# skyhehe123/SA-SSD

Measured on AMD Instinct MI355X. Metric: KITTI-Car inference frames/sec (whole job), higher is better.
Workload: dtype f32; 1 GPU; configs/car_cfg.py inference, fp32, synthetic lidar64 K21 frames (21500 pts -> ~16k voxels), batch=1, random-init SA-SSD weights, points resident in HBM; frames_in_flight=3, spconv_cfg=0, rulebook_pyramid=levels, launch=one hipGraph replay per frame, parallelism=frame-sharded x1, no collective

## Files before the change

### include/sassd.h

```cpp
#ifndef SASSD_H
#define SASSD_H

#include <stddef.h>
#include <stdint.h>

#ifdef __cplusplus
extern "C" {
#endif

#define SASSD_OK       0
#define SASSD_EINVAL  -1
#define SASSD_ENOSPC  -2
#define SASSD_EHIP    -3

#define SASSD_ST_VOXEL_OVERFLOW   1
#define SASSD_ST_HASH_FULL        2
#define SASSD_ST_BOX_OVERFLOW     4
#define SASSD_ST_GRID_SYNC        8

#define SASSD_MAX_POINTS_PER_VOXEL 64

const char *sassd_version(void);
int sassd_last_hip_error(void);
const char *sassd_last_hip_error_string(void);
// ... 88 lines not shown
int sassd_conv2d_wino_supported(int Cin, int Cout, int H, int W);
size_t sassd_conv2d_wino_packed_floats(int Cin, int Cout);
int sassd_conv2d_wino_pack_weight(const float *w, int Cout, int Cin, float *packed, void *stream);
int sassd_conv2d_wino_fwd(const float *x, const float *w_packed, const float *scale, const float *shift, int relu,
                          float *y, int batch, int Cin, int Cout, int H, int W, void *stream);

int sassd_conv2d_wino4_supported(int Cin, int Cout, int H, int W);
size_t sassd_conv2d_wino4_packed_floats(int Cin, int Cout);
int sassd_conv2d_wino4_pack_weight(const float *w , int Cout, int Cin, float *packed, void *stream);
size_t sassd_conv2d_wino4_workspace_bytes(int batch, int Cin, int Cout, int H, int W);
int sassd_conv2d_wino4_fwd(const float *x, const float *w_packed, const float *scale, const float *shift, int relu,
                           float *y, int batch, int Cin, int Cout, int H, int W, int cfg, void *workspace,
                           size_t workspace_bytes, void *stream);

int sassd_conv2d_wino4_chain_supported(int Cin, int Cout, int H, int W);
size_t sassd_conv2d_wino4_chain_workspace_bytes(int batch, int cmax, int H, int W);
int sassd_conv2d_wino4_chain(const float *x, int src_products, const float *prev_scale, const float *prev_shift,
                             int prev_relu, const float *w_packed, const float *scale, const float *shift, int relu,
                             float *y, int batch, int Cin, int Cout, int cmax, int H, int W, const int32_t *tile_map,
                             const int32_t *prev_tile_map, int cfg, void *workspace, size_t workspace_bytes,
                             void *stream);
size_t sassd_conv2d_wino4_narrow_packed_floats(int Cin);
int sassd_conv2d_wino4_pack_weight_narrow(const float *w , int Cout, int Cin, float *packed, void *stream);
int sassd_conv2d_wino4_chain_tail(const float *prev_scale, const float *prev_shift, int prev_relu, float *y_prev,
                                  const float *w_packed64, const float *scale, const float *shift, int relu, float *y,
                                  int batch, int Cin, int Cout, int cmax, int H, int W, const int32_t *prev_tile_map, int cfg,
                                  void *workspace, size_t workspace_bytes, void *stream);

size_t sassd_wino4_tile_map_ints(int batch, int H, int W);
int sassd_wino4_tile_map(const int32_t *indices, const int32_t *n_ptr, int cap, int batch, int H, int W,
                         int32_t *tile_map, void *stream);

int sassd_conv1x1_gemm_supported(int Cin, int Cout, int H, int W);
int sassd_conv1x1_gemm_pack_weight(const float *w , int Cout, int Cin, float *packed, void *stream);
int sassd_conv1x1_gemm_fwd(const float *x, const float *w_packed, const float *scale, const float *shift, int relu,
                           float *y, int batch, int Cin, int Cout, int H, int W, int cfg, void *stream);

int sassd_conv2d_bf16_supported(int Cin, int Cout, int H, int W);
size_t sassd_conv2d_bf16_packed_elems(int Cin, int Cout);
int sassd_conv2d_bf16_pack_weight(const float *w, int Cout, int Cin, void *packed, void *stream);
int sassd_conv2d_bf16_fwd(const float *x, const void *w_packed, const float *shift, float *y, int batch, int Cin,
                          int Cout, int H, int W, void *stream);
int sassd_conv2d_bf16_fwd_cfg(const float *x, const void *w_packed, const float *shift, float *y, int batch, int Cin,
                              int Cout, int H, int W, int cfg, void *stream);
int sassd_conv2d_bf16_bnrelu_fwd(const float *x, const float *in_affine, const void *w_packed, const float *shift, float *y,
                                 int batch, int Cin, int Cout, int H, int W, void *stream);

int sassd_conv1x1_bf16_supported(int Cin, int Cout, int HW);
size_t sassd_conv1x1_bf16_packed_elems(int Cin, int Cout);
int sassd_conv1x1_bf16_pack_weight(const float *w, int Cout, int Cin, int transposed, void *packed, void *stream);
int sassd_conv1x1_bf16_fwd(const float *x, const void *w_packed, const float *shift, float *y, int batch, int Cin, int Cout,
                           int HW, void *stream);

int sassd_conv2d_bf16_infer_supported(int Cin, int Cout, int H, int W);
size_t sassd_conv2d_bf16_infer_packed_elems(int Cin, int Cout);
int sassd_conv2d_bf16_infer_pack_weight(const float *w, int Cout, int Cin, void *packed, void *stream);
int sassd_conv2d_bf16_infer_fwd(const void *x, const void *w_packed, const float *scale, const float *shift, int relu, void *y,
                                int y_bf16, int batch, int Cin, int Cout, int H, int W, void *stream);
int sassd_conv1x1_bf16_infer_supported(int Cin, int Cout, int HW);
int sassd_conv1x1_bf16_infer_fwd(const void *x, const void *w_packed, const float *scale, const float *shift, int relu, void *y,
                                 int y_bf16, int batch, int Cin, int Cout, int HW, void *stream);

size_t sassd_conv2d_wgrad_workspace_bytes(int batch, int Cin, int Cout, int H, int W, int ksize);
int sassd_conv2d_bwd_weight(const float *x, const float *dy, float *dw, int batch, int Cin, int Cout, int H, int W,
                            int ksize, int accumulate, void *workspace, size_t workspace_bytes, void *stream);
int sassd_conv2d_bwd_weight_bf16(const float *x, const float *dy, float *dw, int batch, int Cin, int Cout, int H, int W,
// ... 179 lines not shown
```

### sa-ssd_amd/_C.py

```python
import ctypes as C
import os
import subprocess

_HERE = os.path.dirname(os.path.abspath(__file__))
LIB_PATH = os.path.join(_HERE, "lib", "libsassd.so")
_lib = None

OK, EINVAL, ENOSPC, EHIP = 0, -1, -2, -3
ST_VOXEL_OVERFLOW, ST_HASH_FULL, ST_BOX_OVERFLOW = 1, 2, 4


def build(force=False, verbose=False):
    cmd = ["make", "-C", os.path.join(_HERE, "csrc"), "-j8"]
    if force:
        subprocess.check_call(cmd + ["clean"], stdout=subprocess.DEVNULL)
    out = subprocess.run(cmd, stdout=subprocess.PIPE, stderr=subprocess.STDOUT, text=True)
    if verbose or out.returncode != 0:
        print(out.stdout)
    if out.returncode != 0:
        raise RuntimeError("building libsassd.so failed")
    return LIB_PATH


_SZ = C.c_size_t
# ... 41 lines not shown
    "sassd_conv2d_pack_weight": (_I, [_P, _I, _I, _I, _P, _P]),
    "sassd_conv2d_fwd": (_I, [_P, _P, _P, _P, _I, _P, _I, _I, _I, _I, _I, _I, _P]),
    "sassd_conv2d_fwd_cfg": (_I, [_P, _P, _P, _P, _I, _P, _I, _I, _I, _I, _I, _I, _I, _P]),
    "sassd_anchor_mask_workspace_bytes": (_SZ, [_I, _I]),
    "sassd_anchor_mask": (_I, [_P, _P, _P, _I, _I, _P, _I, _P, _P, _F, _P, _P, _SZ, _P]),
    "sassd_anchor_mask_batch": (_I, [_P, _P, _I, _I, _I, _P, _I, _P, _P, _F, _P, _P, _SZ, _P]),
    "sassd_decode_filter_workspace_bytes": (_SZ, [_I, _I]),
    "sassd_decode_filter": (_I, [_P, _P, _P, _SZ, _I, _I, _I, _I, _I, _P, _P, _F, _P, _P, _P, _P, _I, _P, _P, _SZ, _P]),
    "sassd_pswarp_sample": (_I, [_P, _I, _I, _I, _P, _P, _I, _F, _F, _F, _P, _P]),
    "sassd_pswarp_sample_bwd": (_I, [_P, _I, _I, _I, _P, _P, _I, _F, _F, _F, _P, _P, _P, _P]),
    "sassd_rescore_nms_workspace_bytes": (_SZ, [_I, _I]),
    "sassd_rescore_nms": (_I, [_P, _P, _P, _P, _I, _I, _F, _F, _P, _P, _P, _P, _I, _P, _P, _SZ, _P]),
    "sassd_boxes_overlap_bev": (_I, [_P, _I, _P, _I, _P, _P]),
    "sassd_boxes_iou_bev": (_I, [_P, _I, _P, _I, _P, _P]),
    "sassd_nms_workspace_bytes": (_SZ, [_I]),
    "sassd_nms_gpu": (_I, [_P, _I, _F, _P, _P, _P, _SZ, _P]),
    "sassd_nms_normal_gpu": (_I, [_P, _I, _F, _P, _P, _P, _SZ, _P]),
    "sassd_three_nn": (_I, [_I, _I, _P, _P, _P, _P, _P]),
    "sassd_three_interpolate": (_I, [_I, _I, _I, _P, _P, _P, _P, _P]),
    "sassd_three_interpolate_grad": (_I, [_I, _I, _I, _P, _P, _P, _P, _P]),
    "sassd_pts_in_boxes3d": (_I, [_P, _I, _P, _I, _P, _P, _P]),
    "sassd_three_nn_binned_workspace_bytes": (_SZ, [_I, _I, _I, _I]),
    "sassd_three_nn_binned": (_I, [_I, _I, _P, _P, _F, _F, _F, _I, _I, _I, _P, _P, _P, _SZ, _P]),
    "sassd_conv2d_wino_supported": (_I, [_I, _I, _I, _I]),
    "sassd_conv2d_wino_packed_floats": (_SZ, [_I, _I]),
    "sassd_conv2d_wino_pack_weight": (_I, [_P, _I, _I, _P, _P]),
    "sassd_conv2d_wino_fwd": (_I, [_P, _P, _P, _P, _I, _P, _I, _I, _I, _I, _I, _P]),
    "sassd_conv2d_wino4_supported": (_I, [_I, _I, _I, _I]),
    "sassd_conv2d_wino4_packed_floats": (_SZ, [_I, _I]),
    "sassd_conv2d_wino4_pack_weight": (_I, [_P, _I, _I, _P, _P]),
    "sassd_conv2d_wino4_workspace_bytes": (_SZ, [_I, _I, _I, _I, _I]),
    "sassd_conv2d_wino4_fwd": (_I, [_P, _P, _P, _P, _I, _P, _I, _I, _I, _I, _I, _I, _P, _SZ, _P]),
    "sassd_conv1x1_gemm_supported": (_I, [_I, _I, _I, _I]),
    "sassd_conv1x1_gemm_pack_weight": (_I, [_P, _I, _I, _P, _P]),
    "sassd_conv1x1_narrow_supported": (_I, [_I, _I]),
    "sassd_conv1x1_narrow_pad": (_I, [_I]),
    "sassd_conv1x1_narrow_fwd": (_I, [_P, _P, _P, _P, _I, _P, _I, _I, _I, _I, _I, _P]),
    "sassd_conv1x1_gemm_fwd": (_I, [_P, _P, _P, _P, _I, _P, _I, _I, _I, _I, _I, _I, _P]),
    "sassd_conv2d_bf16_supported": (_I, [_I, _I, _I, _I]),
    "sassd_conv2d_bf16_packed_elems": (_SZ, [_I, _I]),
    "sassd_conv2d_bf16_pack_weight": (_I, [_P, _I, _I, _P, _P]),
    "sassd_conv2d_bf16_fwd": (_I, [_P, _P, _P, _P, _I, _I, _I, _I, _I, _P]),
    "sassd_conv2d_bf16_fwd_cfg": (_I, [_P, _P, _P, _P, _I, _I, _I, _I, _I, _I, _P]),
    "sassd_conv2d_bf16_bnrelu_fwd": (_I, [_P, _P, _P, _P, _P, _I, _I, _I, _I, _I, _P]),
    "sassd_conv1x1_bf16_supported": (_I, [_I, _I, _I]),
    "sassd_conv1x1_bf16_packed_elems": (_SZ, [_I, _I]),
    "sassd_conv1x1_bf16_pack_weight": (_I, [_P, _I, _I, _I, _P, _P]),
    "sassd_conv1x1_bf16_fwd": (_I, [_P, _P, _P, _P, _I, _I, _I, _I, _P]),
    "sassd_conv2d_bf16_infer_supported": (_I, [_I, _I, _I, _I]),
    "sassd_conv2d_bf16_infer_packed_elems": (_SZ, [_I, _I]),
    "sassd_conv2d_bf16_infer_pack_weight": (_I, [_P, _I, _I, _P, _P]),
    "sassd_conv2d_bf16_infer_fwd": (_I, [_P, _P, _P, _P, _I, _P, _I, _I, _I, _I, _I, _I, _P]),
    "sassd_conv1x1_bf16_infer_supported": (_I, [_I, _I, _I]),
    "sassd_conv1x1_bf16_infer_fwd": (_I, [_P, _P, _P, _P, _I, _P, _I, _I, _I, _I, _I, _P]),
    "sassd_conv2d_wgrad_workspace_bytes": (_SZ, [_I, _I, _I, _I, _I, _I]),
    "sassd_conv2d_bwd_weight": (_I, [_P, _P, _P, _I, _I, _I, _I, _I, _I, _I, _P, _SZ, _P]),
    "sassd_assign_targets_workspace_bytes": (_SZ, [_I, _I, _I]),
    "sassd_assign_targets": (_I, [_P, _I, _P, _I, _I, _P, _P, _P, _P, _I, _P, _P, _F, _F, _P, _P, _P, _SZ, _P, _I, _P,
                                  _SZ, _P]),
    "sassd_guided_select_workspace_bytes": (_SZ, [_I, _I]),
    "sassd_guided_select": (_I, [_P, _P, _I, _I, _I, _F, _I, _P, _P, _P, _P, _SZ, _P]),
    "sassd_rpn_loss_workspace_bytes": (_SZ, [_I, _I]),
    "sassd_rpn_loss": (_I, [_P, _P, _P, _I, _P, _P, _P, _I, _P, _I, _I, _P, _P, _P, _P, _P, _SZ, _P]),
    "sassd_conv2d_bwd_weight_bf16": (_I, [_P, _P, _P, _I, _I, _I, _I, _I, _I, _I, _P, _SZ, _P]),
    "sassd_conv2d_bwd_weight_bf16_bnrelu": (_I, [_P, _P, _P, _P, _I, _I, _I, _I, _I, _I, _I, _P, _SZ, _P]),
    "sassd_rotate_iou_eval": (_I, [_P, _I, _P, _I, _I, _P, _P]),
# ... 92 lines not shown
```

### sa-ssd_amd/csrc/conv2d_wino4.hip

```cpp
#include "common.h"

namespace {
typedef float f32x16 __attribute__((ext_vector_type(16)));
typedef __bf16 bf16x8 __attribute__((ext_vector_type(8)));
typedef unsigned u32x4 __attribute__((ext_vector_type(4)));
typedef __attribute__((address_space(3))) void *lds_ptr_t;
typedef const __attribute__((address_space(1))) void *glb_ptr_t;

constexpr int kBM = 128, kKC = 32;

__device__ __forceinline__ void g_row(const float g0, const float g1, const float g2, float (&o)[6])
{
    o[0] = g0;
    const float e = g0 + 0.390625f * g2, f = 0.625f * g1;
    o[1] = e + f;
    o[2] = e - f;
    const float e2 = g0 + 2.25f * g2, f2 = 1.5f * g1;
    o[3] = e2 + f2;
    o[4] = e2 - f2;
    o[5] = g2;
}

__global__ void wino4_pack_kernel(const float *__restrict__ w, int Cout, int Cin, float *__restrict__ U, int ldu)
{
// ... 250 lines not shown
    }
}

static int launch_outin(int dbg, int Cin, int batch, size_t lds, hipStream_t stream, const float *M, W4Geom G,
                        const float *scale, const float *shift, int relu, int pitch, float *V, const int32_t *tmap,
                        float *y_prev)
{
    static std::atomic<unsigned long long> done512{0}, done256{0};
    if (dbg & 256) {
        int rc = sassd_dyn_lds((const void *)wino4_outin_kernel<256>, (size_t)160 * 1024, done256);
        if (rc) return rc;
        hipLaunchKernelGGL(wino4_outin_kernel<256>, dim3(Cin, batch), dim3(256), lds, stream, M, G, scale, shift, relu, pitch,
                           V, tmap, y_prev);
    } else {
        int rc = sassd_dyn_lds((const void *)wino4_outin_kernel<512>, (size_t)160 * 1024, done512);
        if (rc) return rc;
        hipLaunchKernelGGL(wino4_outin_kernel<512>, dim3(Cin, batch), dim3(512), lds, stream, M, G, scale, shift, relu, pitch,
                           V, tmap, y_prev);
    }
    return SASSD_OK;
}

struct W4Gemm {
    const float *U, *V;
    float *M;
    const float *scale, *shift;
    size_t su, sv, sm;
    int np, Cin, Cout, ldv, ldm, ncols, relu;
    int nmb, nnb;
    int nseg, seglen;
    int pairs_per_xcd;
    int dbg;
    const int32_t *ncols_dev;
};

__device__ __forceinline__ void split3(const float a, unsigned &u0, unsigned &u1, unsigned &u2)
{
    u0 = __float_as_uint(a);
    const float r1 = a - __uint_as_float(u0 & 0xffff0000u);
    u1 = __float_as_uint(r1);
    const float r2 = r1 - __uint_as_float(u1 & 0xffff0000u);
    u2 = __float_as_uint(r2);
}
__device__ __forceinline__ unsigned hi_pair(const unsigned lo, const unsigned hi)
{
    return __builtin_amdgcn_perm(hi, lo, 0x07060302u);
}
__device__ __forceinline__ bf16x8 split_a(const float a)
{
    unsigned u0, u1, u2;
    split3(a, u0, u1, u2);
    u32x4 d;
    d[0] = hi_pair(u0, u1); d[1] = hi_pair(u2, u0); d[2] = d[0]; d[3] = hi_pair(u1, u2);
    return __builtin_bit_cast(bf16x8, d);
}
__device__ __forceinline__ bf16x8 split_b(const float w)
{
    unsigned u0, u1, u2;
    split3(w, u0, u1, u2);
    u32x4 d;
    d[0] = hi_pair(u0, u0); d[1] = hi_pair(u0, u1); d[2] = hi_pair(u2, u1); d[3] = d[2];
    return __builtin_bit_cast(bf16x8, d);
}

template <int M, int NM, int NV>
__device__ __forceinline__ void split_sched()
// ... 137 lines not shown
                    for (int a = 0; a < MT; ++a) acc[a][b] = __builtin_amdgcn_mfma_f32_32x32x2f32(av[a], bv, acc[a][b], 0, 0, 0);
                }
            }
        }
        __syncthreads();
    }
    constexpr int WCOLS = 32 * NB;
    float *img = lds + wave * WROWS * WCOLS;
#pragma unroll
    for (int a = 0; a < MT; ++a)
#pragma unroll
        for (int b = 0; b < NB; ++b)
#pragma unroll
            for (int r = 0; r < 16; ++r)
                img[(a * 32 + (r & 3) + 8 * (r >> 2) + 4 * kh) * WCOLS + b * 32 + l31] = acc[a][b][r];
    asm volatile("s_waitcnt lgkmcnt(0)" ::: "memory");
    const int co0 = mb * BM + wm * WROWS;
    float *Mb = P.M + (size_t)p * P.sm + (size_t)co0 * P.ldm + nb * BN + wn * WCOLS;
    constexpr int C4 = WCOLS / 4, RPI = 64 / C4;
    const bool epi = P.scale || P.shift || P.relu;
#pragma unroll
    for (int i = 0; i < WROWS / RPI; ++i) {
        const int row = i * RPI + lane / C4, c4 = lane % C4;
        float4 v = *reinterpret_cast<const float4 *>(img + row * WCOLS + c4 * 4);
        if (epi) {
            const float sc = P.scale ? P.scale[co0 + row] : 1.f, sh = P.shift ? P.shift[co0 + row] : 0.f;
            v.x = v.x * sc + sh; v.y = v.y * sc + sh; v.z = v.z * sc + sh; v.w = v.w * sc + sh;
            if (P.relu) { v.x = fmaxf(v.x, 0.f); v.y = fmaxf(v.y, 0.f); v.z = fmaxf(v.z, 0.f); v.w = fmaxf(v.w, 0.f); }
        }
        *reinterpret_cast<float4 *>(Mb + (size_t)row * P.ldm + c4 * 4) = v;
    }
}

inline int w4_geo(int cfg) { return cfg & 0xff; }
inline int w4_dbg(int cfg) { return cfg >> 8; }

template <int WM, int WN, int NB, int KC, int SPLIT = 0>
int launch_w4_gemm(W4Gemm P, int dbg, hipStream_t stream)
{
    constexpr int BM = 64 * WM, BN = 32 * NB * WN;
    static_assert(BM == kBM || (WM == 1 && SPLIT != 0), "the channel block is fixed (w4_pick_wn and the supported() checks price "
                                                        "it); the one exception is the 64-channel block of a narrow tail layer");
    constexpr size_t stage_b = (size_t)2 * (BM + BN) * KC * 4, img_b = (size_t)WM * WN * 64 * 32 * NB * 4;
    constexpr size_t lds = stage_b > img_b ? stage_b : img_b;
    if constexpr (SPLIT == 1)
        if (dbg & 4) return launch_w4_gemm<WM, WN, NB, KC, 2>(P, dbg, stream);
    static std::atomic<unsigned long long> attr_done{0};
    const void *fn = (const void *)wino4_gemm_kernel<WM, WN, NB, KC, SPLIT>;
    int rc = sassd_dyn_lds(fn, lds, attr_done);
    if (rc) return rc;
    P.nmb = P.Cout / BM; P.nnb = P.ncols / BN;
    const int pairs = P.np * P.nmb;
    P.nseg = pairs >= 32 ? 1 : cdiv(32, pairs);
    if (P.nseg > P.nnb) P.nseg = P.nnb;
    P.seglen = cdiv(P.nnb, P.nseg);
    P.pairs_per_xcd = cdiv(pairs * P.nseg, 8);
    P.dbg = dbg;
    hipLaunchKernelGGL((wino4_gemm_kernel<WM, WN, NB, KC, SPLIT>), dim3(8 * P.pairs_per_xcd * P.seglen), dim3(WM * WN * 64),
                       lds, stream, P);
    return sassd_launch_status();
}

inline int w4_pick_wn(int T, int Cout, int np = 36, bool exact = false)
{
    int best = exact ? 0 : 4;
    double best_cost = 1e30;
    for (int wn = 2; wn <= 6; ++wn) {
        const int bn = 32 * wn;
        if (exact && T % bn) continue;
        const size_t lds = (size_t)2 * (kBM + bn) * kKC * 4;
        int wgs = (int)((size_t)160 * 1024 / lds);
        if (wgs > 32 / (2 * wn)) wgs = 32 / (2 * wn);
        if (wgs < 1) wgs = 1;
        const long units = (long)np * (Cout / kBM) * cdiv(T, bn);
        const long rounds = (units + 256L * wgs - 1) / (256L * wgs);
        const double cost = (double)rounds * wgs * bn;
        if (cost < best_cost - 1e-9) { best_cost = cost; best = wn; }
    }
    return best;
}

struct W4Tile {
    int split, wn, nb, kc;
    int bn() const { return 32 * nb * wn; }
};
inline W4Tile w4_tile(int T, int Cout, int geo)
{
    const int c = geo;
    if (c >= 2 && c <= 6) return W4Tile{0, c, 1, kKC};
    if (c >= 11 && c <= 13) return W4Tile{1, c - 10, 2, kKC};
    if (c == 14) return W4Tile{1, 2, 2, 16};
    if (c == 1) return W4Tile{0, w4_pick_wn(T, Cout), 1, kKC};
    return W4Tile{1, 2, 2, kKC};
}

inline int w4_tiles_padded(int B, int H, int W, int Cout, int geo)
{
    const int T = B * (H / 4) * (W / 4);
    const int bn = w4_tile(T, Cout, geo).bn();
    return cdiv(T, bn) * bn;
}

inline int w4_launch(const W4Tile t, const W4Gemm &P, int dbg, hipStream_t stream)
{
    if (t.split) {
        if (t.kc == 16) return launch_w4_gemm<2, 2, 2, 16, 1>(P, dbg, stream);
        switch (t.wn) {
        case 1: return launch_w4_gemm<2, 1, 2, kKC, 1>(P, dbg, stream);
        case 2: return launch_w4_gemm<2, 2, 2, kKC, 1>(P, dbg, stream);
        default: return launch_w4_gemm<2, 3, 2, kKC, 1>(P, dbg, stream);
        }
    }
    switch (t.wn) {
    case 2: return launch_w4_gemm<2, 2, 1, kKC>(P, dbg, stream);
    case 3: return launch_w4_gemm<2, 3, 1, kKC>(P, dbg, stream);
    case 4: return launch_w4_gemm<2, 4, 1, kKC>(P, dbg, stream);
    case 5: return launch_w4_gemm<2, 5, 1, kKC>(P, dbg, stream);
    default: return launch_w4_gemm<2, 6, 1, kKC>(P, dbg, stream);
    }
}

}

extern "C" int sassd_conv2d_wino4_supported(int Cin, int Cout, int H, int W)
{
    return (Cin >= kKC && Cin % kKC == 0 && Cout >= 256 && Cout % 256 == 0 && H >= 4 && H % 4 == 0 && W >= 4 && W % 4 == 0)
               ? 1 : 0;
}

extern "C" size_t sassd_conv2d_wino4_packed_floats(int Cin, int Cout)
{
    if (Cin < 1 || Cout < 1) return 0;
    return (size_t)36 * Cin * Cout;
}

extern "C" int sassd_conv2d_wino4_pack_weight(const float *w, int Cout, int Cin, float *packed, void *stream_)
{
    if (!w || !packed || Cin < 1 || Cout < 1) return SASSD_EINVAL;
    hipLaunchKernelGGL(wino4_pack_kernel, dim3(cdiv(Cout * Cin, 256)), dim3(256), 0, (hipStream_t)stream_, w, Cout, Cin,
                       packed, Cout);
    return sassd_launch_status();
}

extern "C" size_t sassd_conv2d_wino4_workspace_bytes(int batch, int Cin, int Cout, int H, int W)
{
    if (!sassd_conv2d_wino4_supported(Cin, Cout, H, W) || batch < 1) return 0;
    const size_t Tp = (size_t)cdiv(batch * (H / 4) * (W / 4), 256) * 256 + 256;
    return align_up(36 * (size_t)Cin * Tp * 4, 256) + align_up(36 * (size_t)Cout * Tp * 4, 256);
}

extern "C" int sassd_conv2d_wino4_fwd(const float *x, const float *w_packed, const float *scale, const float *shift,
                                      int relu, float *y, int batch, int Cin, int Cout, int H, int W, int cfg,
                                      void *workspace, size_t workspace_bytes, void *stream_)
{
    if (!x || !w_packed || !y || !workspace || batch < 1 || !sassd_conv2d_wino4_supported(Cin, Cout, H, W))
        return SASSD_EINVAL;
    const int geo = w4_geo(cfg), dbg = w4_dbg(cfg);
    if (((uintptr_t)y & 15) || ((uintptr_t)w_packed & 15) || ((uintptr_t)workspace & 15)) return SASSD_EINVAL;
    if (workspace_bytes < sassd_conv2d_wino4_workspace_bytes(batch, Cin, Cout, H, W)) return SASSD_ENOSPC;
    hipStream_t stream = (hipStream_t)stream_;
    W4Geom G;
    G.B = batch; G.C = Cin; G.H = H; G.W = W; G.TH = H / 4; G.TW = W / 4; G.T = batch * G.TH * G.TW;
    G.Tp = w4_tiles_padded(batch, H, W, Cout, geo);
    float *V = (float *)workspace;
    float *M = (float *)((char *)workspace + align_up(36 * (size_t)Cin * G.Tp * 4, 256));
    if (!(dbg & 16))
        hipLaunchKernelGGL(wino4_in_kernel, dim3(cdiv(G.T, 256), Cin), dim3(256), 0, stream, x, G, V, (const int32_t *)nullptr);
    W4Gemm P;
    P.U = w_packed; P.V = V; P.M = M; P.scale = nullptr; P.shift = nullptr; P.relu = 0; P.ncols_dev = nullptr;
    P.np = 36; P.Cin = Cin; P.Cout = Cout; P.ldv = G.Tp; P.ldm = G.Tp; P.ncols = G.Tp;
    P.su = (size_t)Cin * Cout; P.sv = (size_t)Cin * G.Tp; P.sm = (size_t)Cout * G.Tp;
    int rc = SASSD_OK;
    if (!(dbg & 32)) rc = w4_launch(w4_tile(G.T, Cout, geo), P, dbg, stream);
    if (rc) return rc;
    W4Geom Go = G;
    Go.C = Cout;
    if (!(dbg & 64))
        hipLaunchKernelGGL(wino4_out_kernel, dim3(cdiv(G.T, 256), Cout), dim3(256), 0, stream, (const float *)M, Go, Cout, Cout,
                           scale, shift, relu, y, (const int32_t *)nullptr);
    return sassd_launch_status();
}


namespace {
inline int w4_plane_pitch(int W) { return (W + 2 + 3) / 4 * 4; }
inline size_t w4_plane_bytes(int H, int W) { return (size_t)(H + 2) * w4_plane_pitch(W) * 4; }
}

extern "C" int sassd_conv2d_wino4_chain_supported(int Cin, int Cout, int H, int W)
{
    return sassd_conv2d_wino4_supported(Cin, Cout, H, W) && w4_plane_bytes(H, W) <= (size_t)160 * 1024 ? 1 : 0;
}

extern "C" size_t sassd_conv2d_wino4_chain_workspace_bytes(int batch, int cmax, int H, int W)
{
    if (batch < 1 || cmax < 1 || H < 4 || W < 4 || H % 4 || W % 4) return 0;
    const size_t Tp = (size_t)cdiv(batch * (H / 4) * (W / 4), 256) * 256 + 256;
    return 2 * align_up(36 * (size_t)cmax * Tp * 4, 256);
}

extern "C" int sassd_conv2d_wino4_chain(const float *x, int src_products, const float *prev_scale,
                                        const float *prev_shift, int prev_relu, const float *w_packed,
                                        const float *scale, const float *shift, int relu, float *y, int batch, int Cin,
                                        int Cout, int cmax, int H, int W, const int32_t *tile_map,
                                        const int32_t *prev_tile_map, int cfg, void *workspace,
                                        size_t workspace_bytes, void *stream_)
{
    const int geo = w4_geo(cfg), dbg = w4_dbg(cfg);
    if ((tile_map && src_products) || (prev_tile_map && !src_products)) return SASSD_EINVAL;
    if (!w_packed || !workspace || batch < 1 || !sassd_conv2d_wino4_supported(Cin, Cout, H, W) || cmax < Cin ||
        cmax < Cout || (!src_products && !x))
        return SASSD_EINVAL;
    if (src_products && !sassd_conv2d_wino4_chain_supported(Cin, Cout, H, W)) return SASSD_EINVAL;
    if ((y && ((uintptr_t)y & 15)) || ((uintptr_t)w_packed & 15) || ((uintptr_t)workspace & 15)) return SASSD_EINVAL;
    const size_t need = sassd_conv2d_wino4_chain_workspace_bytes(batch, cmax, H, W);
    if (need == 0 || workspace_bytes < need) return SASSD_ENOSPC;
    hipStream_t stream = (hipStream_t)stream_;
    W4Geom G;
    G.B = batch; G.C = Cin; G.H = H; G.W = W; G.TH = H / 4; G.TW = W / 4; G.T = batch * G.TH * G.TW;
    G.Tp = w4_tiles_padded(batch, H, W, Cout, geo);
    if (src_products && w4_tiles_padded(batch, H, W, Cin, geo) != G.Tp) return SASSD_EINVAL;
    float *V = (float *)workspace;
    float *M = (float *)((char *)workspace + need / 2);
    if (!src_products) {
        if (!(dbg & 16))
            hipLaunchKernelGGL(wino4_in_kernel, dim3(cdiv(G.T, 256), Cin), dim3(256), 0, stream, x, G, V, tile_map);
    } else if (!(dbg & 128)) {
        const size_t lds = w4_plane_bytes(H, W);
        int rc = launch_outin(dbg, Cin, batch, lds, stream, (const float *)M, G, prev_scale, prev_shift, prev_relu,
                              w4_plane_pitch(W), V, prev_tile_map, (float *)nullptr);
        if (rc) return rc;
    }
    W4Gemm P;
    P.U = w_packed; P.V = V; P.M = M; P.scale = nullptr; P.shift = nullptr; P.relu = 0; P.ncols_dev = tile_map;
    P.np = 36; P.Cin = Cin; P.Cout = Cout; P.ldv = G.Tp; P.ldm = G.Tp; P.ncols = G.Tp;
    P.su = (size_t)Cin * Cout; P.sv = (size_t)Cin * G.Tp; P.sm = (size_t)Cout * G.Tp;
    int rc = SASSD_OK;
    if (!(dbg & 32)) rc = w4_launch(w4_tile(G.T, Cout, geo), P, dbg, stream);
    if (rc) return rc;
    if (y && !(dbg & 64)) {
        W4Geom Go = G;
        Go.C = Cout;
        hipLaunchKernelGGL(wino4_out_kernel, dim3(cdiv(G.T, 256), Cout), dim3(256), 0, stream, (const float *)M, Go, Cout, Cout,
                           scale, shift, relu, y, tile_map);
    }
    return sassd_launch_status();
}

extern "C" size_t sassd_conv2d_wino4_narrow_packed_floats(int Cin) { return Cin < 1 ? 0 : (size_t)36 * Cin * 64; }

extern "C" int sassd_conv2d_wino4_pack_weight_narrow(const float *w, int Cout, int Cin, float *packed, void *stream_)
{
    if (!w || !packed || Cin < 1 || Cout < 1 || Cout > 64) return SASSD_EINVAL;
    hipStream_t stream = (hipStream_t)stream_;
    int rc;
    if ((rc = sassd_hip(hipMemsetAsync(packed, 0, sassd_conv2d_wino4_narrow_packed_floats(Cin) * sizeof(float), stream)))) return rc;
    hipLaunchKernelGGL(wino4_pack_kernel, dim3(cdiv(Cout * Cin, 256)), dim3(256), 0, stream, w, Cout, Cin, packed, 64);
    return sassd_launch_status();
}

extern "C" int sassd_conv2d_wino4_chain_tail(const float *prev_scale, const float *prev_shift, int prev_relu, float *y_prev,
                                             const float *w_packed64, const float *scale, const float *shift, int relu,
                                             float *y, int batch, int Cin, int Cout, int cmax, int H, int W,
                                             const int32_t *prev_tile_map, int cfg, void *workspace, size_t workspace_bytes,
                                             void *stream_)
{
    const int geo = w4_geo(cfg), dbg = w4_dbg(cfg);
    if (!w_packed64 || !y || !workspace || batch < 1 || Cout < 1 || Cout > 64 || cmax < Cin || cmax < 64) return SASSD_EINVAL;
    if (!sassd_conv2d_wino4_chain_supported(Cin, 256, H, W) || geo != 0) return SASSD_EINVAL;
    if (((uintptr_t)y & 15) || (y_prev && ((uintptr_t)y_prev & 15)) || ((uintptr_t)w_packed64 & 15) || ((uintptr_t)workspace & 15))
        return SASSD_EINVAL;
    const size_t need = sassd_conv2d_wino4_chain_workspace_bytes(batch, cmax, H, W);
    if (need == 0 || workspace_bytes < need) return SASSD_ENOSPC;
    hipStream_t stream = (hipStream_t)stream_;
    W4Geom G;
    G.B = batch; G.C = Cin; G.H = H; G.W = W; G.TH = H / 4; G.TW = W / 4; G.T = batch * G.TH * G.TW;
    G.Tp = w4_tiles_padded(batch, H, W, 256, geo);
    float *V = (float *)workspace;
    float *M = (float *)((char *)workspace + need / 2);
    int rc;
    if (!(dbg & 128) && (rc = launch_outin(dbg, Cin, batch, w4_plane_bytes(H, W), stream, (const float *)M, G, prev_scale,
                                           prev_shift, prev_relu, w4_plane_pitch(W), V, prev_tile_map, y_prev)))
        return rc;
    W4Gemm P;
    P.U = w_packed64; P.V = V; P.M = M; P.scale = nullptr; P.shift = nullptr; P.relu = 0; P.ncols_dev = nullptr;
    P.np = 36; P.Cin = Cin; P.Cout = 64; P.ldv = G.Tp; P.ldm = G.Tp; P.ncols = G.Tp;
    P.su = (size_t)Cin * 64; P.sv = (size_t)Cin * G.Tp; P.sm = (size_t)64 * G.Tp;
    if (!(dbg & 32) && (rc = launch_w4_gemm<1, 2, 2, kKC, 1>(P, dbg, stream))) return rc;
    W4Geom Go = G;
    Go.C = Cout;
    if (!(dbg & 64))
        hipLaunchKernelGGL(wino4_out_kernel, dim3(cdiv(G.T, 256), Cout), dim3(256), 0, stream, (const float *)M, Go, Cout, 64,
                           scale, shift, relu, y, (const int32_t *)nullptr);
    return sassd_launch_status();
}

namespace {
__global__ void __launch_bounds__(1024) w4_tile_map_kernel(const int32_t *__restrict__ idx, const int32_t *__restrict__ n_ptr,
                                                           int cap, int B, int H, int W, int TH, int TW,
                                                           int32_t *__restrict__ tmap)
{
    extern __shared__ __attribute__((aligned(16))) unsigned char w4_flags[];
    __shared__ int wsum[17];
    const int T = B * TH * TW;
    for (int i = threadIdx.x; i < (T + 3) / 4; i += 1024) ((unsigned *)w4_flags)[i] = 0u;
    __syncthreads();
    const int n = min(*n_ptr, cap);
    for (int r = threadIdx.x; r < n; r += 1024) {
        const int4 c = ((const int4 *)idx)[r];
        if (c.x < 0 || c.x >= B || c.z < 0 || c.z >= H || c.w < 0 || c.w >= W) continue;
        const int ty = c.z >> 2, tx = c.w >> 2;
        const int y0 = ((c.z & 3) == 0 && ty > 0) ? ty - 1 : ty, y1 = ((c.z & 3) == 3 && ty + 1 < TH) ? ty + 1 : ty;
        const int x0 = ((c.w & 3) == 0 && tx > 0) ? tx - 1 : tx, x1 = ((c.w & 3) == 3 && tx + 1 < TW) ? tx + 1 : tx;
        for (int a = y0; a <= y1; ++a)
            for (int e = x0; e <= x1; ++e) w4_flags[(c.x * TH + a) * TW + e] = 1;
    }
    __syncthreads();
    const int per = (T + 1023) / 1024;
// ... 15 lines not shown
{
    if (batch < 1 || H < 4 || W < 4 || H % 4 || W % 4) return 0;
    const size_t T = (size_t)batch * (H / 4) * (W / 4);
    return T <= 65536 ? kTmapHead + 2 * T : 0;
}

extern "C" int sassd_wino4_tile_map(const int32_t *indices, const int32_t *n_ptr, int cap, int batch, int H, int W,
                                    int32_t *tile_map, void *stream_)
{
    if (!indices || !n_ptr || !tile_map || cap < 1 || sassd_wino4_tile_map_ints(batch, H, W) == 0) return SASSD_EINVAL;
    const int TH = H / 4, TW = W / 4, T = batch * TH * TW;
    hipLaunchKernelGGL(w4_tile_map_kernel, dim3(1), dim3(1024), (size_t)align_up((size_t)T, 16), (hipStream_t)stream_, indices,
                       n_ptr, cap, batch, H, W, TH, TW, tile_map);
    return sassd_launch_status();
}


namespace {
__global__ void conv1x1_pack_kernel(const float *__restrict__ w, int Cout, int Cin, float *__restrict__ U)
{
    const int i = blockIdx.x * blockDim.x + threadIdx.x;
    if (i >= Cout * Cin) return;
    const int co = i % Cout, ci = i / Cout;
    U[(size_t)ci * Cout + co] = w[(size_t)co * Cin + ci];
}
}

extern "C" int sassd_conv1x1_gemm_supported(int Cin, int Cout, int H, int W)
{
    if (!(Cin >= kKC && Cin % kKC == 0 && Cout >= kBM && Cout % kBM == 0 && H > 0 && W > 0)) return 0;
    return w4_pick_wn(H * W, Cout, 1, true) ? 1 : 0;
}

extern "C" int sassd_conv1x1_gemm_pack_weight(const float *w, int Cout, int Cin, float *packed, void *stream_)
{
    if (!w || !packed || Cin < 1 || Cout < 1) return SASSD_EINVAL;
    hipLaunchKernelGGL(conv1x1_pack_kernel, dim3(cdiv(Cout * Cin, 256)), dim3(256), 0, (hipStream_t)stream_, w, Cout, Cin,
                       packed);
    return sassd_launch_status();
}

extern "C" int sassd_conv1x1_gemm_fwd(const float *x, const float *w_packed, const float *scale, const float *shift,
                                      int relu, float *y, int batch, int Cin, int Cout, int H, int W, int cfg,
                                      void *stream_)
{
    if (!x || !w_packed || !y || batch < 1 || !sassd_conv1x1_gemm_supported(Cin, Cout, H, W)) return SASSD_EINVAL;
    const int geo = w4_geo(cfg), dbg = w4_dbg(cfg);
    if (((uintptr_t)y & 15) || ((uintptr_t)w_packed & 15) || ((uintptr_t)x & 15)) return SASSD_EINVAL;
    const int hw = H * W;
    W4Gemm P;
    P.U = w_packed; P.V = x; P.M = y; P.scale = scale; P.shift = shift; P.relu = relu; P.ncols_dev = nullptr;
    P.np = batch; P.Cin = Cin; P.Cout = Cout; P.ldv = hw; P.ldm = hw; P.ncols = hw;
    P.su = 0; P.sv = (size_t)Cin * hw; P.sm = (size_t)Cout * hw;
    hipStream_t stream = (hipStream_t)stream_;
    if (geo != 1 && hw % 128 == 0) return launch_w4_gemm<2, 2, 2, kKC, 1>(P, dbg, stream);
    switch (w4_pick_wn(hw, Cout, batch, true)) {
    case 2: return launch_w4_gemm<2, 2, 1, kKC>(P, dbg, stream);
    case 3: return launch_w4_gemm<2, 3, 1, kKC>(P, dbg, stream);
    case 4: return launch_w4_gemm<2, 4, 1, kKC>(P, dbg, stream);
    case 5: return launch_w4_gemm<2, 5, 1, kKC>(P, dbg, stream);
    case 6: return launch_w4_gemm<2, 6, 1, kKC>(P, dbg, stream);
    }
    return SASSD_EINVAL;
}
```

### sa-ssd_amd/kernels.py

```python
import numpy as np
import torch

from . import _C

_ws_cache = {}

_weights_gen = [0]


def weights_generation():
    return _weights_gen[0]


def bump_weights_generation():
    _weights_gen[0] += 1


def weight_key(w):
    return (w._version, w.data_ptr(), str(w.device), _weights_gen[0])


_ws_scope = [None]


# ... 508 lines not shown
                                               _C.stream()), "sassd_conv2d_wino4_chain")
    return y


def conv2d_wino4_pack_weight_narrow(w):
    _chk_cuda(w)
    cout, cin = w.shape[0], w.shape[1]
    L = _C.lib()
    packed = torch.empty(L.sassd_conv2d_wino4_narrow_packed_floats(cin), dtype=torch.float32, device=w.device)
    _C.check(L.sassd_conv2d_wino4_pack_weight_narrow(_C.ptr(w.contiguous()), cout, cin, _C.ptr(packed), _C.stream()),
             "sassd_conv2d_wino4_pack_weight_narrow")
    return packed


def conv2d_wino4_chain_tail(prev, y_prev, w_packed64, cin, cout, cmax, batch, h, w, scale, shift, relu, y, ws, cfg=None,
                            prev_tile_map=None):
    _chk_cuda(w_packed64, scale, shift, y, ws, y_prev)
    ps, pb, pr = prev
    _C.check(_C.lib().sassd_conv2d_wino4_chain_tail(_C.ptr(ps), _C.ptr(pb), 1 if pr else 0, _C.ptr(y_prev), _C.ptr(w_packed64),
                                                    _C.ptr(scale), _C.ptr(shift), 1 if relu else 0, _C.ptr(y), batch, cin, cout,
                                                    cmax, h, w, _C.ptr(prev_tile_map),
                                                    DEFAULT_CFG["wino4"] if cfg is None else int(cfg), _C.ptr(ws), ws.numel(),
                                                    _C.stream()), "sassd_conv2d_wino4_chain_tail")
    return y


def conv1x1_gemm_supported(cin, cout, h, w):
    return bool(_C.lib().sassd_conv1x1_gemm_supported(int(cin), int(cout), int(h), int(w)))


def conv1x1_gemm_pack_weight(w):
    _chk_cuda(w)
    cout, cin = w.shape[0], w.shape[1]
    packed = torch.empty(cin * cout, dtype=torch.float32, device=w.device)
    _C.check(_C.lib().sassd_conv1x1_gemm_pack_weight(_C.ptr(w.contiguous()), cout, cin, _C.ptr(packed), _C.stream()),
             "sassd_conv1x1_gemm_pack_weight")
    return packed


def conv1x1_gemm_fwd(x, w_packed, cout, scale=None, shift=None, relu=False, y=None, cfg=None):
    _chk_cuda(x, w_packed, scale, shift)
    b, cin, h, w = x.shape
    if y is None:
        y = torch.empty(b, cout, h, w, dtype=torch.float32, device=x.device)
    _C.check(_C.lib().sassd_conv1x1_gemm_fwd(_C.ptr(x), _C.ptr(w_packed), _C.ptr(scale), _C.ptr(shift), 1 if relu else 0,
                                             _C.ptr(y), b, cin, cout, h, w,
                                             DEFAULT_CFG["wino4"] if cfg is None else int(cfg), _C.stream()),
             "sassd_conv1x1_gemm_fwd")
    return y


def conv2d_bf16_supported(cin, cout, h, w):
    return bool(_C.lib().sassd_conv2d_bf16_supported(cin, cout, h, w))


def conv2d_bf16_pack_weight(w):
    _chk_cuda(w)
    cout, cin, kh, kw = w.shape
    assert kh == 3 and kw == 3
    L = _C.lib()
    packed = torch.empty(L.sassd_conv2d_bf16_packed_elems(cin, cout), dtype=torch.int16, device=w.device)
    _C.check(L.sassd_conv2d_bf16_pack_weight(_C.ptr(w.contiguous()), cout, cin, _C.ptr(packed), _C.stream()),
             "sassd_conv2d_bf16_pack_weight")
    return packed


def conv2d_bf16_fwd(x, w_packed, cout, shift=None, y=None, in_affine=None, cfg=0):
# ... 647 lines not shown
```

Baseline: 946.5 frames/s.

## Add pre-split bf16 weight planes GEMM kernel for wino4 and 1x1 convs

Adds a new 256x128-tile GEMM kernel for the Winograd F(4,3) and 1x1 conv paths. Weights are pre-split once at pack time into three bf16 planes appended after the fp32 weights, so per-call splitting only happens on the activation side. The kernel runs eight 3-plane bf16 MFMA products to emulate fp32 and double-buffers staging through LDS with direct global-to-LDS loads. It becomes the default tile choice for geo 0, which costs extra weight memory and a larger LDS footprint per block.

Result: slower. 891.3 frames/s (-5.8%).

```diff
diff --git a/include/sassd.h b/include/sassd.h
--- a/include/sassd.h
+++ b/include/sassd.h
@@ -144,6 +144,7 @@
                          int32_t *tile_map, void *stream);
 
 int sassd_conv1x1_gemm_supported(int Cin, int Cout, int H, int W);
+size_t sassd_conv1x1_gemm_packed_floats(int Cin, int Cout);
 int sassd_conv1x1_gemm_pack_weight(const float *w , int Cout, int Cin, float *packed, void *stream);
 int sassd_conv1x1_gemm_fwd(const float *x, const float *w_packed, const float *scale, const float *shift, int relu,
                            float *y, int batch, int Cin, int Cout, int H, int W, int cfg, void *stream);
diff --git a/sa-ssd_amd/_C.py b/sa-ssd_amd/_C.py
--- a/sa-ssd_amd/_C.py
+++ b/sa-ssd_amd/_C.py
@@ -97,6 +97,7 @@
     "sassd_conv2d_wino4_workspace_bytes": (_SZ, [_I, _I, _I, _I, _I]),
     "sassd_conv2d_wino4_fwd": (_I, [_P, _P, _P, _P, _I, _P, _I, _I, _I, _I, _I, _I, _P, _SZ, _P]),
     "sassd_conv1x1_gemm_supported": (_I, [_I, _I, _I, _I]),
+    "sassd_conv1x1_gemm_packed_floats": (_SZ, [_I, _I]),
     "sassd_conv1x1_gemm_pack_weight": (_I, [_P, _I, _I, _P, _P]),
     "sassd_conv1x1_narrow_supported": (_I, [_I, _I]),
     "sassd_conv1x1_narrow_pad": (_I, [_I]),
diff --git a/sa-ssd_amd/csrc/conv2d_wino4.hip b/sa-ssd_amd/csrc/conv2d_wino4.hip
--- a/sa-ssd_amd/csrc/conv2d_wino4.hip
+++ b/sa-ssd_amd/csrc/conv2d_wino4.hip
@@ -306,6 +306,8 @@
     int pairs_per_xcd;
     int dbg;
     const int32_t *ncols_dev;
+    const unsigned short *Up;
+    size_t sup;
 };
 
 __device__ __forceinline__ void split3(const float a, unsigned &u0, unsigned &u1, unsigned &u2)
@@ -509,6 +511,186 @@
     }
 }
 
+template <int KC, int OVL, int NOSPLIT>
+__global__ void __launch_bounds__(512) wino4_gemm_planes_kernel(W4Gemm P)
+{
+    constexpr int BM = 256, BN = 128, G8 = KC / 8;
+    constexpr int A_B = 3 * G8 * BM * 16, B32_B = KC * BN * 4, BP_B = 3 * G8 * BN * 16;
+    constexpr int NLA = A_B / 1024, NLB = B32_B / 1024;
+    static_assert(NLA % 8 == 0 && NLB % 8 == 0, "every wave issues the same loads");
+    extern __shared__ __attribute__((aligned(16))) unsigned char w4p_lds[];
+    unsigned char *const As = w4p_lds, *const B32 = As + 2 * A_B, *const Bp = B32 + 2 * B32_B;
+    const int tid = threadIdx.x, lane = tid & 63;
+    const int wave = __builtin_amdgcn_readfirstlane(tid >> 6);
+    const int xcd = blockIdx.x & 7, j = blockIdx.x >> 3;
+    const int q = j / P.seglen, within = j - q * P.seglen;
+    const int item = xcd * P.pairs_per_xcd + q;
+    if (item >= P.np * P.nmb * P.nseg) return;
+    const int pair = item / P.nseg, nb = (item - pair * P.nseg) * P.seglen + within;
+    if (nb >= P.nnb) return;
+    if (P.ncols_dev && nb * BN >= *P.ncols_dev) return;
+    const int p = pair / P.nmb, mb = pair - p * P.nmb;
+    const size_t pstride = (size_t)(P.Cin / 8) * P.Cout * 8;
+    const unsigned short *Ub = P.Up + (size_t)p * P.sup + (size_t)mb * BM * 8;
+    const float *Vb = P.V + (size_t)p * P.sv + nb * BN;
+    unsigned offa[NLA / 8], offb[NLB / 8];
+#pragma unroll
+    for (int i = 0; i < NLA / 8; ++i) {
+        const int t = wave + 8 * i, pg = t >> 2, qt = t & 3;
+        offa[i] = (unsigned)(((size_t)(pg / G8) * pstride + ((size_t)(pg % G8) * P.Cout + qt * 64 + lane) * 8) * 2);
+    }
+#pragma unroll
+    for (int i = 0; i < NLB / 8; ++i) {
+        const int e = (wave + 8 * i) * 64 + lane;
+        offb[i] = (unsigned)(((size_t)(e >> 5) * P.ldv + (e & 31) * 4) * 4);
+    }
+    const unsigned ka = (unsigned)G8 * P.Cout * 16, kb = (unsigned)KC * P.ldv * 4;
+    auto dma_a = [&](int chunk, int st) {
+        unsigned adv = chunk * ka;
+        asm volatile("" : "+s"(adv));
+        const char *base = reinterpret_cast<const char *>(Ub) + adv;
+#pragma unroll
+        for (int i = 0; i < NLA / 8; ++i)
+            __builtin_amdgcn_global_load_lds((glb_ptr_t)(base + offa[i]), (lds_ptr_t)(As + st * A_B + (wave + 8 * i) * 1024), 16, 0, 0);
+    };
+    auto dma_b = [&](int chunk, int st) {
+        unsigned adv = chunk * kb;
+        asm volatile("" : "+s"(adv));
+        const char *base = reinterpret_cast<const char *>(Vb) + adv;
+#pragma unroll
+        for (int i = 0; i < NLB / 8; ++i)
+            __builtin_amdgcn_global_load_lds((glb_ptr_t)(base + offb[i]), (lds_ptr_t)(B32 + st * B32_B + (wave + 8 * i) * 1024), 16, 0,
+                                             0);
+    };
+    const int scol = tid & 127, sq = wave >> 1;
+    auto split_pass = [&](int st, int pb) {
+        const float *src = (const float *)(B32 + st * B32_B) + scol;
+        unsigned char *dst = Bp + pb * BP_B + scol * 16;
+#pragma unroll
+        for (int qq = 0; qq < KC / 16; ++qq) {
+            const int k4 = sq + 4 * qq;
+            unsigned u[4][3];
+#pragma unroll
+            for (int i = 0; i < 4; ++i) split3(src[(4 * k4 + i) * BN], u[i][0], u[i][1], u[i][2]);
+#pragma unroll
+            for (int pc = 0; pc < 3; ++pc)
+                *reinterpret_cast<uint2 *>(dst + (pc * G8 + (k4 >> 1)) * (BN * 16) + (k4 & 1) * 8) =
+                    make_uint2(hi_pair(u[0][pc], u[1][pc]), hi_pair(u[2][pc], u[3][pc]));
+        }
+    };
+    const int wm = wave & 3, wn = wave >> 2;
+    const int l31 = lane & 31, kh = lane >> 5;
+    f32x16 acc[2][2];
+#pragma unroll
+    for (int a = 0; a < 2; ++a)
+#pragma unroll
+        for (int b = 0; b < 2; ++b)
+#pragma unroll
+            for (int r = 0; r < 16; ++r) acc[a][b][r] = 0.f;
+    const int aoff = (kh * BM + wm * 64 + l31) * 16, boff = (kh * BN + wn * 64 + l31) * 16;
+    auto mfma_block = [&](int st, int pb) {
+        const unsigned char *Ac = As + st * A_B + aoff, *Bc = Bp + pb * BP_B + boff;
+#pragma unroll
+        for (int s = 0; s < KC / 16; ++s) {
+            bf16x8 af[3][2], bfr[3][2];
+#pragma unroll
+            for (int pc = 0; pc < 3; ++pc)
+#pragma unroll
+                for (int t = 0; t < 2; ++t) {
+                    af[pc][t] = *reinterpret_cast<const bf16x8 *>(Ac + ((pc * G8 + 2 * s) * BM + 32 * t) * 16);
+                    bfr[pc][t] = *reinterpret_cast<const bf16x8 *>(Bc + ((pc * G8 + 2 * s) * BN + 32 * t) * 16);
+                }
+            constexpr int PA[8] = {1, 2, 0, 2, 1, 0, 1, 0}, PB[8] = {2, 1, 2, 0, 1, 1, 0, 0};
+#pragma unroll
+            for (int ps = 0; ps < 8; ++ps)
+#pragma unroll
+                for (int b = 0; b < 2; ++b)
+#pragma unroll
+                    for (int a = 0; a < 2; ++a)
+                        acc[a][b] = __builtin_amdgcn_mfma_f32_32x32x16_bf16(af[PA[ps]][a], bfr[PB[ps]][b], acc[a][b], 0, 0, 0);
+        }
+    };
+    const int nchunk = P.Cin / KC;
+    const bool stage_all = !(P.dbg & 1);
+    if constexpr (OVL) {
+        dma_a(0, 0);
+        dma_b(0, 0);
+        if (nchunk > 1) dma_b(1, 1);
+        __syncthreads();
+        if constexpr (!NOSPLIT) split_pass(0, 0);
+        __syncthreads();
+        for (int c = 0; c < nchunk; ++c) {
+            if constexpr (!NOSPLIT)
+                if (c + 1 < nchunk) split_pass((c + 1) & 1, (c + 1) & 1);
+            if (c + 1 < nchunk && stage_all) dma_a(c + 1, (c + 1) & 1);
+            if (c + 2 < nchunk && stage_all) dma_b(c + 2, c & 1);
+            mfma_block(c & 1, c & 1);
+            __syncthreads();
+        }
+    } else {
+        dma_a(0, 0);
+        dma_b(0, 0);
+        __syncthreads();
+        for (int c = 0; c < nchunk; ++c) {
+            if constexpr (!NOSPLIT) split_pass(c & 1, 0);
+            if (c + 1 < nchunk && stage_all) { dma_a(c + 1, (c + 1) & 1); dma_b(c + 1, (c + 1) & 1); }
+            asm volatile("s_waitcnt lgkmcnt(0)\n\ts_barrier" ::: "memory");
+            mfma_block(c & 1, 0);
+            __syncthreads();
+        }
+    }
+    float *img = reinterpret_cast<float *>(w4p_lds) + wave * 64 * 64;
+#pragma unroll
+    for (int a = 0; a < 2; ++a)
+#pragma unroll
+        for (int b = 0; b < 2; ++b)
+#pragma unroll
+            for (int r = 0; r < 16; ++r)
+                img[(a * 32 + (r & 3) + 8 * (r >> 2) + 4 * kh) * 64 + b * 32 + l31] = acc[a][b][r];
+    asm volatile("s_waitcnt lgkmcnt(0)" ::: "memory");
+    const int co0 = mb * BM + wm * 64;
+    float *Mb = P.M + (size_t)p * P.sm + (size_t)co0 * P.ldm + nb * BN + wn * 64;
+    const bool epi = P.scale || P.shift || P.relu;
+#pragma unroll
+    for (int i = 0; i < 16; ++i) {
+        const int row = i * 4 + (lane >> 4), c4 = lane & 15;
+        float4 v = *reinterpret_cast<const float4 *>(img + row * 64 + c4 * 4);
+        if (epi) {
+            const float sc = P.scale ? P.scale[co0 + row] : 1.f, sh = P.shift ? P.shift[co0 + row] : 0.f;
+            v.x = v.x * sc + sh; v.y = v.y * sc + sh; v.z = v.z * sc + sh; v.w = v.w * sc + sh;
+            if (P.relu) { v.x = fmaxf(v.x, 0.f); v.y = fmaxf(v.y, 0.f); v.z = fmaxf(v.z, 0.f); v.w = fmaxf(v.w, 0.f); }
+        }
+        *reinterpret_cast<float4 *>(Mb + (size_t)row * P.ldm + c4 * 4) = v;
+    }
+}
+
+__global__ void wino4_pieces_kernel(const float *__restrict__ U, int np, int Cin, int Cout, unsigned short *__restrict__ Up)
+{
+    const size_t i = (size_t)blockIdx.x * blockDim.x + threadIdx.x;
+    const int c8n = Cin / 8;
+    if (i >= (size_t)np * c8n * Cout) return;
+    const int co = (int)(i % Cout), c8 = (int)(i / Cout % c8n), p = (int)(i / Cout / c8n);
+    unsigned u[8][3];
+#pragma unroll
+    for (int k = 0; k < 8; ++k) split3(U[((size_t)p * Cin + c8 * 8 + k) * Cout + co], u[k][0], u[k][1], u[k][2]);
+#pragma unroll
+    for (int pc = 0; pc < 3; ++pc) {
+        u32x4 d;
+#pragma unroll
+        for (int k = 0; k < 4; ++k) d[k] = hi_pair(u[2 * k][pc], u[2 * k + 1][pc]);
+        *reinterpret_cast<u32x4 *>(Up + ((((size_t)p * 3 + pc) * c8n + c8) * Cout + co) * 8) = d;
+    }
+}
+inline size_t w4_piece_floats(size_t n, int Cin) { return Cin % 8 == 0 ? n * 3 / 2 : 0; }
+inline int w4_write_pieces(float *packed, int np, int Cin, int Cout, hipStream_t stream)
+{
+    if (Cin % 8) return SASSD_OK;
+    const size_t n = (size_t)np * (Cin / 8) * Cout;
+    hipLaunchKernelGGL(wino4_pieces_kernel, dim3((unsigned)((n + 255) / 256)), dim3(256), 0, stream, (const float *)packed, np,
+                       Cin, Cout, reinterpret_cast<unsigned short *>(packed + (size_t)np * Cin * Cout));
+    return sassd_launch_status();
+}
+
 inline int w4_geo(int cfg) { return cfg & 0xff; }
 inline int w4_dbg(int cfg) { return cfg >> 8; }
 
@@ -538,6 +720,32 @@
     return sassd_launch_status();
 }
 
+template <int KC, int OVL, int NOSPLIT = 0>
+int launch_w4_planes(W4Gemm P, int dbg, hipStream_t stream)
+{
+    if constexpr (!NOSPLIT)
+        if (dbg & 4) return launch_w4_planes<KC, OVL, 1>(P, dbg, stream);
+    constexpr int G8 = KC / 8;
+    constexpr size_t stage_b = (size_t)2 * 3 * G8 * 256 * 16 + (size_t)2 * KC * 128 * 4 + (size_t)(1 + OVL) * 3 * G8 * 128 * 16;
+    constexpr size_t img_b = (size_t)8 * 64 * 64 * 4;
+    constexpr size_t lds = stage_b > img_b ? stage_b : img_b;
+    static_assert(lds <= (size_t)160 * 1024, "the staging buffers fit a CU's LDS");
+    if (!P.Up || P.Cin % KC || P.Cout % 256 || P.ncols % 128) return SASSD_EINVAL;
+    if ((size_t)P.Cin * P.Cout * 6 >= ((size_t)1 << 31) || (size_t)P.Cin * P.ldv * 4 >= ((size_t)1 << 31)) return SASSD_EINVAL;
+    static std::atomic<unsigned long long> attr_done{0};
+    int rc = sassd_dyn_lds((const void *)wino4_gemm_planes_kernel<KC, OVL, NOSPLIT>, lds, attr_done);
+    if (rc) return rc;
+    P.nmb = P.Cout / 256; P.nnb = P.ncols / 128;
+    const int pairs = P.np * P.nmb;
+    P.nseg = pairs >= 32 ? 1 : cdiv(32, pairs);
+    if (P.nseg > P.nnb) P.nseg = P.nnb;
+    P.seglen = cdiv(P.nnb, P.nseg);
+    P.pairs_per_xcd = cdiv(pairs * P.nseg, 8);
+    P.dbg = dbg;
+    hipLaunchKernelGGL((wino4_gemm_planes_kernel<KC, OVL, NOSPLIT>), dim3(8 * P.pairs_per_xcd * P.seglen), dim3(512), lds, stream, P);
+    return sassd_launch_status();
+}
+
 inline int w4_pick_wn(int T, int Cout, int np = 36, bool exact = false)
 {
     int best = exact ? 0 : 4;
@@ -559,16 +767,18 @@
 
 struct W4Tile {
     int split, wn, nb, kc;
+    int planes;
     int bn() const { return 32 * nb * wn; }
 };
 inline W4Tile w4_tile(int T, int Cout, int geo)
 {
     const int c = geo;
-    if (c >= 2 && c <= 6) return W4Tile{0, c, 1, kKC};
-    if (c >= 11 && c <= 13) return W4Tile{1, c - 10, 2, kKC};
-    if (c == 14) return W4Tile{1, 2, 2, 16};
-    if (c == 1) return W4Tile{0, w4_pick_wn(T, Cout), 1, kKC};
-    return W4Tile{1, 2, 2, kKC};
+    if (c >= 2 && c <= 6) return W4Tile{0, c, 1, kKC, 0};
+    if (c >= 11 && c <= 13) return W4Tile{1, c - 10, 2, kKC, 0};
+    if (c == 14) return W4Tile{1, 2, 2, 16, 0};
+    if (c == 1) return W4Tile{0, w4_pick_wn(T, Cout), 1, kKC, 0};
+    if (c >= 21 && c <= 23) return W4Tile{1, 2, 2, c == 22 ? 32 : 16, c - 20};
+    return W4Tile{1, 2, 2, 16, 1};
 }
 
 inline int w4_tiles_padded(int B, int H, int W, int Cout, int geo)
@@ -580,6 +790,11 @@
 
 inline int w4_launch(const W4Tile t, const W4Gemm &P, int dbg, hipStream_t stream)
 {
+    switch (t.planes) {
+    case 1: return launch_w4_planes<16, 1>(P, dbg, stream);
+    case 2: return launch_w4_planes<32, 0>(P, dbg, stream);
+    case 3: return launch_w4_planes<16, 0>(P, dbg, stream);
+    }
     if (t.split) {
         if (t.kc == 16) return launch_w4_gemm<2, 2, 2, 16, 1>(P, dbg, stream);
         switch (t.wn) {
@@ -608,7 +823,8 @@
 extern "C" size_t sassd_conv2d_wino4_packed_floats(int Cin, int Cout)
 {
     if (Cin < 1 || Cout < 1) return 0;
-    return (size_t)36 * Cin * Cout;
+    const size_t n = (size_t)36 * Cin * Cout;
+    return n + w4_piece_floats(n, Cin);
 }
 
 extern "C" int sassd_conv2d_wino4_pack_weight(const float *w, int Cout, int Cin, float *packed, void *stream_)
@@ -616,7 +832,8 @@
     if (!w || !packed || Cin < 1 || Cout < 1) return SASSD_EINVAL;
     hipLaunchKernelGGL(wino4_pack_kernel, dim3(cdiv(Cout * Cin, 256)), dim3(256), 0, (hipStream_t)stream_, w, Cout, Cin,
                        packed, Cout);
-    return sassd_launch_status();
+    int rc = sassd_launch_status();
+    return rc ? rc : w4_write_pieces(packed, 36, Cin, Cout, (hipStream_t)stream_);
 }
 
 extern "C" size_t sassd_conv2d_wino4_workspace_bytes(int batch, int Cin, int Cout, int H, int W)
@@ -645,6 +862,7 @@
         hipLaunchKernelGGL(wino4_in_kernel, dim3(cdiv(G.T, 256), Cin), dim3(256), 0, stream, x, G, V, (const int32_t *)nullptr);
     W4Gemm P;
     P.U = w_packed; P.V = V; P.M = M; P.scale = nullptr; P.shift = nullptr; P.relu = 0; P.ncols_dev = nullptr;
+    P.Up = reinterpret_cast<const unsigned short *>(w_packed + (size_t)36 * Cin * Cout); P.sup = (size_t)3 * Cin * Cout;
     P.np = 36; P.Cin = Cin; P.Cout = Cout; P.ldv = G.Tp; P.ldm = G.Tp; P.ncols = G.Tp;
     P.su = (size_t)Cin * Cout; P.sv = (size_t)Cin * G.Tp; P.sm = (size_t)Cout * G.Tp;
     int rc = SASSD_OK;
@@ -710,6 +928,7 @@
     }
     W4Gemm P;
     P.U = w_packed; P.V = V; P.M = M; P.scale = nullptr; P.shift = nullptr; P.relu = 0; P.ncols_dev = tile_map;
+    P.Up = reinterpret_cast<const unsigned short *>(w_packed + (size_t)36 * Cin * Cout); P.sup = (size_t)3 * Cin * Cout;
     P.np = 36; P.Cin = Cin; P.Cout = Cout; P.ldv = G.Tp; P.ldm = G.Tp; P.ncols = G.Tp;
     P.su = (size_t)Cin * Cout; P.sv = (size_t)Cin * G.Tp; P.sm = (size_t)Cout * G.Tp;
     int rc = SASSD_OK;
@@ -744,7 +963,8 @@
 {
     const int geo = w4_geo(cfg), dbg = w4_dbg(cfg);
     if (!w_packed64 || !y || !workspace || batch < 1 || Cout < 1 || Cout > 64 || cmax < Cin || cmax < 64) return SASSD_EINVAL;
-    if (!sassd_conv2d_wino4_chain_supported(Cin, 256, H, W) || geo != 0) return SASSD_EINVAL;
+    if (!sassd_conv2d_wino4_chain_supported(Cin, 256, H, W) || w4_tile(batch * (H / 4) * (W / 4), 256, geo).bn() != 128)
+        return SASSD_EINVAL;
     if (((uintptr_t)y & 15) || (y_prev && ((uintptr_t)y_prev & 15)) || ((uintptr_t)w_packed64 & 15) || ((uintptr_t)workspace & 15))
         return SASSD_EINVAL;
     const size_t need = sassd_conv2d_wino4_chain_workspace_bytes(batch, cmax, H, W);
@@ -761,6 +981,7 @@
         return rc;
     W4Gemm P;
     P.U = w_packed64; P.V = V; P.M = M; P.scale = nullptr; P.shift = nullptr; P.relu = 0; P.ncols_dev = nullptr;
+    P.Up = nullptr; P.sup = 0;
     P.np = 36; P.Cin = Cin; P.Cout = 64; P.ldv = G.Tp; P.ldm = G.Tp; P.ncols = G.Tp;
     P.su = (size_t)Cin * 64; P.sv = (size_t)Cin * G.Tp; P.sm = (size_t)64 * G.Tp;
     if (!(dbg & 32) && (rc = launch_w4_gemm<1, 2, 2, kKC, 1>(P, dbg, stream))) return rc;
@@ -842,12 +1063,20 @@
     return w4_pick_wn(H * W, Cout, 1, true) ? 1 : 0;
 }
 
+extern "C" size_t sassd_conv1x1_gemm_packed_floats(int Cin, int Cout)
+{
+    if (Cin < 1 || Cout < 1) return 0;
+    const size_t n = (size_t)Cin * Cout;
+    return n + w4_piece_floats(n, Cin);
+}
+
 extern "C" int sassd_conv1x1_gemm_pack_weight(const float *w, int Cout, int Cin, float *packed, void *stream_)
 {
     if (!w || !packed || Cin < 1 || Cout < 1) return SASSD_EINVAL;
     hipLaunchKernelGGL(conv1x1_pack_kernel, dim3(cdiv(Cout * Cin, 256)), dim3(256), 0, (hipStream_t)stream_, w, Cout, Cin,
                        packed);
-    return sassd_launch_status();
+    int rc = sassd_launch_status();
+    return rc ? rc : w4_write_pieces(packed, 1, Cin, Cout, (hipStream_t)stream_);
 }
 
 extern "C" int sassd_conv1x1_gemm_fwd(const float *x, const float *w_packed, const float *scale, const float *shift,
@@ -862,7 +1091,12 @@
     P.U = w_packed; P.V = x; P.M = y; P.scale = scale; P.shift = shift; P.relu = relu; P.ncols_dev = nullptr;
     P.np = batch; P.Cin = Cin; P.Cout = Cout; P.ldv = hw; P.ldm = hw; P.ncols = hw;
     P.su = 0; P.sv = (size_t)Cin * hw; P.sm = (size_t)Cout * hw;
+    P.Up = reinterpret_cast<const unsigned short *>(w_packed + (size_t)Cin * Cout); P.sup = 0;
     hipStream_t stream = (hipStream_t)stream_;
+    if (hw % 128 == 0 && Cout % 256 == 0) {
+        const W4Tile t = w4_tile(hw, Cout, geo);
+        if (t.planes) return w4_launch(t, P, dbg, stream);
+    }
     if (geo != 1 && hw % 128 == 0) return launch_w4_gemm<2, 2, 2, kKC, 1>(P, dbg, stream);
     switch (w4_pick_wn(hw, Cout, batch, true)) {
     case 2: return launch_w4_gemm<2, 2, 1, kKC>(P, dbg, stream);
diff --git a/sa-ssd_amd/kernels.py b/sa-ssd_amd/kernels.py
--- a/sa-ssd_amd/kernels.py
+++ b/sa-ssd_amd/kernels.py
@@ -564,7 +564,7 @@
 def conv1x1_gemm_pack_weight(w):
     _chk_cuda(w)
     cout, cin = w.shape[0], w.shape[1]
-    packed = torch.empty(cin * cout, dtype=torch.float32, device=w.device)
+    packed = torch.empty(_C.lib().sassd_conv1x1_gemm_packed_floats(cin, cout), dtype=torch.float32, device=w.device)
     _C.check(_C.lib().sassd_conv1x1_gemm_pack_weight(_C.ptr(w.contiguous()), cout, cin, _C.ptr(packed), _C.stream()),
              "sassd_conv1x1_gemm_pack_weight")
     return packed
```
